# cerbos/cerbos

Measured on NVIDIA H100. Metric: checkresources_decisions_per_sec, higher is better.
Workload: dtype u64

## Files before the change

### cerbos_b200/csrc/cb_core.h

```cpp
#pragma once
#include <stdint.h>
#if !defined(__CUDACC_RTC__)
#include <math.h>
#endif

#include "cerbos_b200_format.h"

#if defined(__CUDACC__)
#define CB_HD __host__ __device__ __forceinline__
#define CB_HD_NOINLINE __host__ __device__ __noinline__
#else
#define CB_HD inline
#define CB_HD_NOINLINE
#endif

namespace cb {

struct alignas(16) U4 { uint32_t x, y, z, w; };

struct TableLayout {
    uint32_t off[32];
    uint32_t nV, nRP, nS, nP, nR, nAP, nT, n_slots, n_rows;
    uint32_t has_role_policies, has_parent_roles, has_principal_policies;
    uint32_t image_bytes;
    uint32_t uc_conds_off, uc_rows_off, uc_chain_off, n_uconds;
    uint32_t theap_words;
    uint32_t uses_runtime;
};

struct TableView {
    const uint8_t *base;
    const TableLayout *L;
    template <typename T>
    CB_HD const T *sec(int id) const { return reinterpret_cast<const T *>(base + L->off[id]); }
    CB_HD const uint32_t *scope_parent() const { return sec<uint32_t>(CB_SEC_SCOPE_PARENT); }
    CB_HD const uint32_t *scope_flags() const { return sec<uint32_t>(CB_SEC_SCOPE_FLAGS); }
    CB_HD const uint32_t *res_block_map() const { return sec<uint32_t>(CB_SEC_RES_BLOCK_MAP); }
    CB_HD const uint8_t *res_exists() const { return sec<uint8_t>(CB_SEC_RES_EXISTS); }
    CB_HD const uint32_t *prin_block_map() const { return sec<uint32_t>(CB_SEC_PRIN_BLOCK_MAP); }
    CB_HD const uint8_t *prin_exists() const { return sec<uint8_t>(CB_SEC_PRIN_EXISTS); }
// ... 9 lines not shown
    CB_HD const uint8_t *str_bytes() const { return sec<uint8_t>(CB_SEC_STR_BYTES); }
    CB_HD const uint32_t *par_off() const { return sec<uint32_t>(CB_SEC_ROLE_PARENTS_OFF); }
    CB_HD const uint32_t *par_list() const { return sec<uint32_t>(CB_SEC_ROLE_PARENTS); }
    CB_HD const uint32_t *rp_off() const { return sec<uint32_t>(CB_SEC_ROLEPOL_OFF); }
    CB_HD const cb_rolepol_entry *rp_entries() const { return sec<cb_rolepol_entry>(CB_SEC_ROLEPOL_ENTRIES); }
    CB_HD const cb_rolepol_rule *rp_rules() const { return sec<cb_rolepol_rule>(CB_SEC_ROLEPOL_RULES); }
    CB_HD const uint32_t *rp_apats() const { return sec<uint32_t>(CB_SEC_ROLEPOL_APATS); }
    CB_HD const uint32_t *block_slots_off() const { return sec<uint32_t>(CB_SEC_BLOCK_SLOTS_OFF); }
    CB_HD const uint32_t *block_slots() const { return sec<uint32_t>(CB_SEC_BLOCK_SLOTS); }
    CB_HD const uint32_t *dr_off() const { return sec<uint32_t>(CB_SEC_DR_OFF); }
    CB_HD const uint32_t *dr_entries() const { return sec<uint32_t>(CB_SEC_DR_ENTRIES); }
    CB_HD const uint32_t *dr_parents() const { return sec<uint32_t>(CB_SEC_DR_PARENTS); }
    CB_HD const uint32_t *dr_name_str() const { return sec<uint32_t>(CB_SEC_DR_NAME_STR); }
    CB_HD const cb_cond *uconds() const { return reinterpret_cast<const cb_cond *>(base + L->uc_conds_off); }
    CB_HD const U4 *urows() const { return reinterpret_cast<const U4 *>(base + L->uc_rows_off); }
    CB_HD const U4 *uc_chain() const { return reinterpret_cast<const U4 *>(base + L->uc_chain_off); }
};

enum { CB_MAX_GATHER = 8 };
struct BatchView {
    const cb_hdr0 *hdr0;
    const cb_hdr1 *hdr1;
    const uint32_t *roles;
    const uint64_t *slots;
    const uint64_t *heap;
    const uint32_t *bstr_off;
    const uint8_t *bstr_bytes;
    const uint32_t *class_off, *class_pats, *aset_k;
    const uint64_t *aset_spread;
    const uint64_t *row_am;
// ... 4223 lines not shown
        for (uint32_t j = 1; j < RC; j++) x |= allow_pairs >> j;
        x &= amask;
        if (RC == 1) acc = x;
        else if (RC == 2) { x = (x | x >> 1) & 0x33333333u; x = (x | x >> 2) & 0x0F0F0F0Fu; x = (x | x >> 4) & 0x00FF00FFu; acc = (x | x >> 8) & 0xFFFFu; }
        else for (uint32_t kk = 0; kk < K; kk++) acc |= ((x >> (kk * RC)) & 1) << kk;
    }
    store_result(b, cols, n, bitmap, effects, K, acc);
    return false;
}

CB_HD U4 uc_row_record(const U4 ur, uint32_t am, uint32_t RCP, uint32_t nR) {
    const uint32_t role = ur.y & 0xFFu, deny = ((ur.y >> 8) & 0xFFu) == CB_EFFECT_DENY;
    U4 r; r.x = am; r.y = ur.z; r.z = ur.w; r.w = (role == 0xFFu ? nR : role) * RCP | deny << 31;
    return r;
}
struct UcRowsGlobal {
    const U4 *urows; const uint64_t *row_am; uint32_t RCP, nR;
    CB_HD U4 get(uint32_t aset_base, uint32_t ri) const { const U4 ur = ld16(urows + ri); return uc_row_record(ur, (uint32_t)ldg(row_am + aset_base + ur.x), RCP, nR); }
};
struct UcRowsPacked {
    const U4 *pk;
    CB_HD U4 get(uint32_t aset_base, uint32_t ri) const { return ld16(pk + aset_base + ri); }
};

struct CachedCols {
    const BatchView *b;
    uint64_t n;
    CB_HD U4 hdr0() const { return ldcol128(b->hdr0 + n); }
    CB_HD uint64_t hdr1() const { return ldcol64(reinterpret_cast<const uint64_t *>(b->hdr1 + n)); }
    CB_HD uint32_t role(uint32_t i) const { return ldcol32(b->roles + (uint64_t)i * b->stride + n); }
    CB_HD uint64_t slot(uint32_t v) const {
#if defined(__CUDA_ARCH__)
        uint64_t x;
        asm("ld.global.nc.u64 %0, [%1];" : "=l"(x) : "l"(b->slots + (uint64_t)v * b->stride + n));
        return x;
#else
        return b->slots[(uint64_t)v * b->stride + n];
#endif
    }
    CB_HD void prefetch_slot(uint32_t) const {}
    CB_HD bool staged() const { return true; }
    CB_HD uint32_t aset_k(uint32_t aset) const { return ldg(b->aset_k + aset); }
    CB_HD const uint64_t *row_am() const { return b->row_am; }
    CB_HD bool stage_result(uint32_t) const { return false; }
};

struct CondWord { uint64_t lo, hi; };
enum { CB_UC_FORM_MASK32 = 0, CB_UC_FORM_MASK64 = 1, CB_UC_FORM_INDEX = 2 };
struct GenericConds {
    static constexpr int kForm = CB_UC_FORM_MASK64;
    static constexpr uint32_t kScopeRows = 0;
    template <typename Cols>
    CB_HD Cols load(const TableView, const BatchView &, const Cols &cols) const { return cols; }
    template <typename Cols>
    CB_HD CondWord operator()(const TableView t, const BatchView &b, const Cols &cols, uint32_t pid, uint64_t n, bool &slow) const {
        if (t.L->n_uconds > 63) { slow = true; CondWord w; w.lo = 1; w.hi = 0; return w; }
        uint64_t val = 1;
        for (uint32_t u = 1, nu = t.L->n_uconds; u <= nu; u++) {
            const U4 cd = ld16(t.uconds() + u);
            uint32_t r;
            if (cd.w) r = flat_dnf_inline(t, b, cols, pid, cd.z, cd.w);
            else r = 4u;
            slow |= (r & 4u) != 0;
            val |= (uint64_t)(r & 1u) << u;
        }
        CondWord w; w.lo = val; w.hi = 0;
        return w;
    }
};

CB_HD uint32_t cond_bit(const CondWord v, uint32_t u) { return (uint32_t)(((u & 64u) ? v.hi : v.lo) >> (u & 63u)) & 1u; }
template <typename RP, int kForm>
CB_HD uint32_t uc_row_pairs(const U4 r, const RP rp, const CondWord v, const uint32_t role_all) {
    const uint32_t vlo = (uint32_t)v.lo, vhi = (uint32_t)(v.lo >> 32);
    const uint32_t miss = kForm == CB_UC_FORM_MASK32   ? r.y & ~vlo
                          : kForm == CB_UC_FORM_MASK64 ? (r.y & ~vlo) | (r.z & ~vhi)
                                                       : (cond_bit(v, r.y & 0xFFu) & cond_bit(v, (r.y >> 8) & 0xFFu)) ^ 1u;
    const uint32_t rc = miss ? 0u : (uint32_t)(rp >> (r.w & (sizeof(RP) * 8 - 1))) & role_all;
    return r.x * rc;
}
constexpr uint32_t kUcUnrollRows = 16;
template <uint32_t kRows, typename RP, int kForm, typename Rows>
CB_HD uint32_t uc_walk(const TableView t, const Rows rows, const RP rp, const CondWord val, const uint32_t r0, const uint32_t bm_base,
                       const uint32_t aset_base, const uint32_t role_all, uint32_t alive) {
    uint32_t allow_pairs = 0;
    const U4 *chain = t.uc_chain() + bm_base;
    for (uint32_t s = r0; s != CB_NONE32 && alive;) {
        const U4 d = ld16(chain + s);
        uint32_t D = 0, A = 0;
        auto row = [&](uint32_t ri) {
            const U4 r = rows.get(aset_base, ri);
            const uint32_t p = uc_row_pairs<RP, kForm>(r, rp, val, role_all), deny = (uint32_t)((int32_t)r.w >> 31);
            D |= p & deny;
            A |= p & ~deny;
        };
        if constexpr (kRows != 0 && kRows <= kUcUnrollRows) {
            if (d.x < d.z) {
                const uint32_t last = d.z - d.x - 1;
#if defined(__CUDA_ARCH__)
#pragma unroll
#endif
                for (uint32_t j = 0; j < kRows; j++) row(d.x + (j < last ? j : last));
            }
        } else {
#if defined(__CUDA_ARCH__)
#pragma unroll 4
#endif
            for (uint32_t ri = d.x; ri < d.z; ri++) row(ri);
        }
        D &= alive;
        alive &= ~D;
        A &= alive;
        allow_pairs |= A;
        alive &= ~A;
        s = d.w;
    }
    return allow_pairs;
}

template <typename Cols, typename Rows, typename Conds = GenericConds>
CB_HD bool eval_request_uc(const TableView t, const BatchView &b, const Cols &cols, const Rows rows, uint64_t n, uint8_t *bitmap, uint8_t *effects,
                           const Conds conds = Conds()) {
    const U4 h0 = cols.hdr0();
// ... 11 lines not shown
        rp |= rr < t.L->nR ? 1ull << (rr * RCP + i) : 0ull;
    }
    if (pv != rv) return true;
    uint32_t acc = 0;
    const bool live = n_roles != 0 && K != 0 && rv != CB_NONE16 && kc != CB_KIND_NONE;
#ifdef CB_UC_STUB_WALK
    const uint32_t r0 = live ? rscope & 0xFFFFu : CB_NONE32;
#else
    const uint32_t r0 = live ? chain_start(t, rscope, CB_SCOPE_FLAG_RESOURCE, (b.flags & CB_BATCH_FLAG_LENIENT) != 0) : CB_NONE32;
#endif
    if (r0 != CB_NONE32) {
        bool slow = false;
        const CondWord val = conds(t, b, regs, pid, n, slow);
        if (slow) return true;
        const uint32_t role_all = (1u << n_roles) - 1;
        const uint32_t aset_base = aset * b.n_rows;
        const uint32_t amask = K * RC >= 32 ? b.stride_pattern : b.stride_pattern & ((1u << (K * RC)) - 1);
        const uint32_t alive0 = amask * role_all;
        const uint32_t bm_base = (rv * t.L->nRP + kc) * t.L->nS;
        uint32_t allow_pairs;
#ifdef CB_UC_STUB_WALK
        allow_pairs = alive0 & ((uint32_t)val.lo ^ (uint32_t)(val.lo >> 32) ^ (uint32_t)rp ^ r0 ^ bm_base ^ aset_base);
        (void)rows;
#else
        if ((t.L->nR + 1) * RCP <= 32)
            allow_pairs = uc_walk<Conds::kScopeRows, uint32_t, Conds::kForm>(t, rows, (uint32_t)rp | role_all << (t.L->nR * RCP), val, r0, bm_base, aset_base, role_all, alive0);
        else allow_pairs = uc_walk<Conds::kScopeRows, uint64_t, Conds::kForm>(t, rows, rp | (uint64_t)role_all << (t.L->nR * RCP), val, r0, bm_base, aset_base, role_all, alive0);
#endif
        uint32_t x = allow_pairs;
        x |= RC > 1 ? allow_pairs >> 1 : 0u;
        x |= RC > 2 ? allow_pairs >> 2 : 0u;
        x |= RC > 3 ? allow_pairs >> 3 : 0u;
        for (uint32_t j = 4; j < RC; j++) x |= allow_pairs >> j;
        x &= amask;
        if (RC == 1) acc = x;
        else if (RC == 2) { x = (x | x >> 1) & 0x33333333u; x = (x | x >> 2) & 0x0F0F0F0Fu; x = (x | x >> 4) & 0x00FF00FFu; acc = (x | x >> 8) & 0xFFFFu; }
        else if (RC == 3) { x = (x | x >> 2) & 0xC30C30C3u; x = (x | x >> 4) & 0x0F00F00Fu; x = (x | x >> 8) & 0xFF0000FFu; acc = (x | x >> 16) & 0x7FFu; }
        else if (RC == 4) { x = (x | x >> 3) & 0x03030303u; x = (x | x >> 6) & 0x000F000Fu; acc = (x | x >> 12) & 0xFFu; }
        else for (uint32_t kk = 0; kk < K; kk++) acc |= ((x >> (kk * RC)) & 1) << kk;
    }
    store_result(b, cols, n, bitmap, effects, K, acc);
    return false;
// ... 13 lines not shown
```

### cerbos_b200/csrc/cb_host.h

```cpp
#pragma once
#include <cstdarg>
#include <cstdint>
#include <cstdio>
#include <cstring>
#include <string>

#include "cb_core.h"
#include "cb_uc.h"
#include "cerbos_b200.h"

namespace cbhost {

constexpr int kMaxSec = 32;

inline std::string msg(const char *fmt, ...) {
    char buf[512];
    va_list ap;
    va_start(ap, fmt);
    vsnprintf(buf, sizeof(buf), fmt, ap);
    va_end(ap);
    return buf;
}

inline std::string parse_blob(const void *blob, size_t len, cb::TableLayout *lay, uint32_t *meta, uint64_t *sec_len) {
// ... 90 lines not shown
    cb::finish_batch_view(*v);
    v->n_bstr = cb_[CGPU_COL_BSTR_OFF] >= 4 ? (uint32_t)(cb_[CGPU_COL_BSTR_OFF] / 4 - 1) : 0;
    v->heap_words = cb_[CGPU_COL_HEAP] / 8;
    return "";
}


inline bool lean_table(const cb::TableLayout &lay, const uint32_t *meta) {
    return !lay.has_principal_policies && !lay.has_role_policies && !lay.has_parent_roles && meta[CB_META_DIRECT_KINDS];
}
inline bool lean_eligible(const cb::TableLayout &lay, const uint32_t *meta, const cb::BatchView &bv) {
    return bv.n_pass == 1 && (uint64_t)bv.max_actions * bv.role_cols <= 32 && bv.kbytes <= 4 && lean_table(lay, meta) &&
           (uint64_t)lay.nR * bv.rcp <= 64;
}
inline bool uc_eligible(const cb::TableLayout &lay, const cbuc::Image &uc, const cb::BatchView &bv) {
    return uc.ok && (uint64_t)(lay.nR + 1) * bv.rcp <= 64 && bv.count < (1ull << 32) && (uint64_t)bv.n_asets * lay.n_rows < (1ull << 31);
}

}
```

### cerbos_b200/csrc/cb_kernels.h

```cpp
#pragma once
#include "cb_core.h"

namespace cbk {

constexpr int kThreads = 256;

struct TableDesc {
    const uint8_t *base;
    cb::TableLayout lay;
};

__device__ __forceinline__ uint32_t smem_u32(const void *p) { return (uint32_t)__cvta_generic_to_shared(p); }

__device__ __forceinline__ void mbar_wait(uint64_t *bar, uint32_t parity) {
    uint32_t ok = 0;
    while (!ok) {
        asm volatile("{\n\t.reg .pred p;\n\tmbarrier.try_wait.parity.shared::cta.b64 p, [%1], %2;\n\tselp.u32 %0, 1, 0, p;\n\t}"
                     : "=r"(ok)
                     : "r"(smem_u32(bar)), "r"(parity)
                     : "memory");
    }
}
__device__ __forceinline__ void mbar_init(uint64_t *bar, uint32_t count) { asm volatile("mbarrier.init.shared::cta.b64 [%0], %1;" ::"r"(smem_u32(bar)), "r"(count)); }
__device__ __forceinline__ void mbar_expect_tx(uint64_t *bar, uint32_t bytes) {
// ... 230 lines not shown
        else if (q < 6 + bv.role_cols) { p = (unsigned long long)(bv.roles + (uint64_t)(q - 6) * bv.stride); sh = 2; }
        else { const uint32_t v = q - 6 - bv.role_cols; p = (unsigned long long)(bv.slots + (uint64_t)(v >> 1) * bv.stride) + (v & 1u) * 128u; sh = 3; }
        pf_base[q] = p;
        pf_shift[q] = sh;
    }
    if (!kStaged) __syncthreads();
    if (kStaged) {
        if (threadIdx.x == 0) {
            mbar_init(mbar, 1);
            asm volatile("fence.mbarrier_init.release.cluster;" ::: "memory");
        }
        __syncthreads();
        if (threadIdx.x == 0) tma_load_image(smem_image, td, mbar);
        mbar_wait(mbar, 0);
        cb::U4 *pks = reinterpret_cast<cb::U4 *>(smem_image + ((td.lay.image_bytes + 127u) & ~127u));
        const uint32_t n_pk = bv.n_asets * bv.n_rows;
        const cb::U4 *ur = tv.urows();
        for (uint32_t j = threadIdx.x; j < n_pk; j += kThreads) {
            const cb::U4 u = ur[j % bv.n_rows];
            pks[j] = cb::uc_row_record(u, (uint32_t)bv.row_am[(j / bv.n_rows) * bv.n_rows + u.x], bv.rcp, td.lay.nR);
        }
        __syncthreads();
        pk = pks;
    }
    const uint32_t lane = threadIdx.x & 31u;
    const uint64_t n_chunks = (bv.count + 31) / 32;
    const uint64_t n_warps = (uint64_t)gridDim.x * (kThreads / 32);
    for (uint64_t chunk = (uint64_t)blockIdx.x * (kThreads / 32) + (threadIdx.x >> 5); chunk < n_chunks; chunk += n_warps) {
        const uint64_t i = chunk * 32 + lane;
        {
            const uint64_t c2 = chunk + n_warps;
            if (c2 * 32 + 32 <= bv.count) {
                const uint64_t n2 = bv.first + c2 * 32;
                for (uint32_t q = lane; q < n_pf; q += 32) asm volatile("prefetch.global.L2 [%0];" ::"l"(pf_base[q] + (n2 << pf_shift[q])));
            }
        }
        if (i < bv.count) {
            const uint64_t n = bv.first + i;
            Cols gc;
            gc.b = &bv; gc.n = n;
            bool d;
            if (kStaged || pk) { cb::UcRowsPacked rows; rows.pk = pk; d = cb::eval_request_uc(tv, bv, gc, rows, n, bitmap, effects, Conds()); }
            else { cb::UcRowsGlobal rows; rows.urows = tv.urows(); rows.row_am = bv.row_am; rows.RCP = bv.rcp; rows.nR = td.lay.nR; d = cb::eval_request_uc(tv, bv, gc, rows, n, bitmap, effects, Conds()); }
            if (d) {
                cb::store_result(bv, gc, n, bitmap, effects, bv.max_actions, 0u);
                const uint32_t k = atomicAdd(bv.defer_count, 1u);
                bv.defer_list[k] = (uint32_t)i;
            }
        }
    }
}

}
```

### cerbos_b200/csrc/cb_specialize.h

```cpp
#pragma once
#include <stdint.h>

#include <cstdio>
#include <cstring>
#include <map>
#include <string>
#include <vector>

#include "cerbos_b200_format.h"

namespace cbspec {

struct Limits {
    uint32_t max_shapes = 8;
    uint32_t max_items = 96;
};

inline std::string hex(uint32_t v) {
    char buf[16];
    snprintf(buf, sizeof buf, "0x%xu", v);
    return buf;
}
inline std::string hex64(uint64_t v) {
    char buf[32];
// ... 374 lines not shown
    uint32_t max_terms = 512;
};
struct UcSource {
    std::string src;
    uint32_t n_strpred = 0;
    uint32_t n_atoms = 0;
};
inline UcSource generate_uc(const uint8_t *uc_image, const uint32_t *off, uint32_t uc_conds_off, uint32_t n_uconds, uint32_t n_slots, uint32_t n_consts = 0,
                            const UcLimits lim = UcLimits()) {
    UcSource out;
    if (n_uconds == 0 || n_uconds > 127) return out;
    const uint32_t *const_words = reinterpret_cast<const uint32_t *>(uc_image + off[CB_SEC_CONSTS]);
    Atoms atoms;
    std::vector<std::string> formula(n_uconds + 1);
    const uint32_t *uconds = reinterpret_cast<const uint32_t *>(uc_image + uc_conds_off);
    const uint32_t scope_rows = uconds[0];
    const uint32_t *code = reinterpret_cast<const uint32_t *>(uc_image + off[CB_SEC_CODE]);
    const uint64_t *consts = reinterpret_cast<const uint64_t *>(uc_image + off[CB_SEC_CONSTS_V64]);
    const uint64_t *theap = reinterpret_cast<const uint64_t *>(uc_image + off[CB_SEC_THEAP]);
    const uint32_t kUseMask = ~((uint32_t)(CB_TERM_LIT_F | CB_TERM_GROUP_END) << 8);
    std::map<std::vector<uint32_t>, uint32_t> term_ids;
    std::vector<std::vector<uint32_t>> terms;
    const uint32_t ns = n_slots ? n_slots : 1;
    std::vector<bool> slot_used(ns, false), slot_list(ns, false);
    auto is_slot_kind = [](uint32_t kind) { return kind == CB_OPK_SLOT || kind == CB_OPK_SLOT_ELEM || kind == CB_OPK_SLOT_SIZE; };
    auto use_slot = [&](uint32_t kind, uint32_t v) { if (is_slot_kind(kind) && v < ns) slot_used[v] = true; };
    auto v64_tag = [](uint64_t b) { const uint32_t top = (uint32_t)(b >> 48); return (top & 0xFFF0u) == 0xFFF0u ? (top & 0xFu) : 0u; };
    for (uint32_t u = 1; u <= n_uconds; u++) {
        const uint32_t *cd = uconds + 4 * u;
        if (cd[3] == 0 || ((cd[3] >> 16) & 0xFF) != CB_FLAT_DNF) {
            formula[u] = translate_program(code, cd[0], cd[1], const_words, n_consts, ns, atoms);
// ... 284 lines not shown
        for (uint32_t v = 0; v < ns; v++) {
            const std::string V = std::to_string(v);
            if (ty[v] == 'S') s += "    ListKey k" + V + ";   // string: its probe key (the id when typed)\n";
            if (ty[v] == 'N') s += "    double d" + V + ";\n";
            if (ty[v] == 'B') s += "    bool b" + V + ";\n";
        }
    }
    for (uint32_t v = 0; v < ns; v++)
        if (slot_list[v]) s += "    ListRegs l" + std::to_string(v) + ";\n";
    s += "    CB_HD uint64_t slot(uint32_t v) const {\n        switch (v) {\n";
    for (uint32_t v = 0; v < ns && !typed; v++)
        if (reg(v)) s += "        case " + std::to_string(v) + "u: return s" + std::to_string(v) + ";\n";
    s += "        default: return v < " + std::to_string(ns) + "u ? g.slot(v) : (uint64_t)(CB_V64_BOX_BASE | CB_V64_ERROR) << 48;\n        }\n    }\n};\n";
    s += "struct SpecConds {\n    static constexpr uint32_t n_strpred = " + std::to_string(n_pred_bits) + "u;\n";
    s += std::string("    static constexpr int kForm = ") + (n_uconds <= 31 ? "CB_UC_FORM_MASK32" : n_uconds <= 63 ? "CB_UC_FORM_MASK64" : "CB_UC_FORM_INDEX") + ";   // how the rows name their conditions\n";
    s += "    static constexpr uint32_t kScopeRows = " + std::to_string(scope_rows) + "u;   // rows of the longest scope (cb::uc_walk)\n";
    s += std::string("    static constexpr bool kPrograms = ") + (have_atoms ? "true" : "false") + ";   // leaf programs: needs the value helpers of cb_core.h\n";
    s += "    template <typename Cols>\n    CB_HD SpecRegs load(const TableView t, const BatchView &b, const Cols &c) const {\n        SpecRegs r;\n        r.g.b = c.b; r.g.n = c.n;\n";
    for (uint32_t v = 0; v < ns; v++)
        if (reg(v)) s += "        r.s" + std::to_string(v) + " = c.slot(" + std::to_string(v) + "u);\n";
    if (typed) {
        std::string guard;
        for (uint32_t v = 0; v < ns; v++) {
            const std::string V = std::to_string(v);
            if (!reg(v)) continue;
            if (ty[v] == 'L') s += "        r.l" + V + " = list_load(t, b, r.s" + V + ");\n";
            if (ty[v] == 'S') s += "        r.k" + V + " = list_probe_key(r.s" + V + ");\n";
            if (ty[v] == 'N') s += "        r.d" + V + " = u2d(r.s" + V + ");\n";
            if (ty[v] == 'B') s += "        r.b" + V + " = (r.s" + V + " & 1u) != 0;\n";
            guard += std::string(guard.empty() ? "" : " & ") + (ty[v] == 'L' ? "typed_list(r.l" + V + ", " + std::to_string(list_need[v]) + "u)"
                                                                 : std::string(ty[v] == 'S' ? "typed_str" : ty[v] == 'N' ? "typed_num" : "typed_bool") + "(r.s" + V + ")");
// ... 117 lines not shown
```

### cerbos_b200/csrc/cb_uc.h

```cpp
#pragma once
#include <stdint.h>

#include <cstring>
#include <map>
#include <string>
#include <tuple>
#include <vector>

#include "cb_core.h"

namespace cbuc {

constexpr uint32_t kMaxUconds = 127;
constexpr uint32_t kMaxMaskUconds = 63;

struct Image {
    bool ok = false;
    std::string why;
    std::vector<uint8_t> bytes;
    cb::TableLayout lay{};
    uint32_t n_uconds = 0, n_flat = 0;
    bool needs_spec() const { return n_flat != n_uconds || n_uconds > kMaxMaskUconds; }
    uint32_t scope_rows = 0;
    uint32_t n_gids = 0, n_gids_flat = 0;
    std::vector<uint32_t> ucond_of_gid;
};

inline Image build(const uint8_t *image, const uint32_t *off, const uint64_t *len, const uint32_t *meta, const cb::TableLayout &lay) {
    Image out;
    const uint32_t n_blocks = meta[CB_META_N_BLOCKS], n_rows = meta[CB_META_N_ROWS], n_conds = meta[CB_META_N_CONDS];
    if (n_blocks == 0) { out.why = "no policy blocks"; return out; }
    if (lay.nR > 64) { out.why = "more than 64 roles"; return out; }
    const uint32_t *blocks = reinterpret_cast<const uint32_t *>(image + off[CB_SEC_BLOCKS]);
    const uint32_t *rows = reinterpret_cast<const uint32_t *>(image + off[CB_SEC_ROWS]);
    const uint32_t *conds = reinterpret_cast<const uint32_t *>(image + off[CB_SEC_CONDS]);
    if (len[CB_SEC_BLOCKS] < (uint64_t)n_blocks * 16 || len[CB_SEC_ROWS] < (uint64_t)n_rows * 16 || len[CB_SEC_CONDS] < (uint64_t)n_conds * 16) {
        out.why = "section sizes do not match META";
        return out;
// ... 50 lines not shown
    const uint64_t n_map = (uint64_t)meta[CB_META_N_VERSIONS] * meta[CB_META_N_RESPATS] * nS;
    if (nS == 0 || len[CB_SEC_SCOPE_PARENT] < (uint64_t)nS * 4 || len[CB_SEC_SCOPE_FLAGS] < (uint64_t)nS * 4 || len[CB_SEC_RES_BLOCK_MAP] < n_map * 4) {
        out.why = "scope tables do not match the block map";
        return out;
    }
    const uint32_t *parent = reinterpret_cast<const uint32_t *>(image + off[CB_SEC_SCOPE_PARENT]);
    const uint32_t *sflags = reinterpret_cast<const uint32_t *>(image + off[CB_SEC_SCOPE_FLAGS]);
    const uint32_t *bmap = reinterpret_cast<const uint32_t *>(image + off[CB_SEC_RES_BLOCK_MAP]);
    std::vector<uint32_t> next(nS);
    for (uint32_t s = 0; s < nS; s++) {
        uint32_t x = s, steps = 0;
        do { x = parent[x]; } while (x != CB_NONE32 && x < nS && ++steps <= nS && !(sflags[x] & CB_SCOPE_FLAG_RESOURCE));
        if (x != CB_NONE32 && (x >= nS || steps > nS)) { out.why = "scope parent chain out of range"; return out; }
        next[s] = x;
    }
    std::vector<uint32_t> chain(4 * (size_t)n_map, 0);
    for (uint64_t e = 0; e < n_map; e++) {
        const uint32_t s = (uint32_t)(e % nS), bid = bmap[e];
        uint32_t *d = chain.data() + 4 * e;
        if (bid != CB_NONE32) {
            if (bid >= n_blocks) { out.why = "block map entry out of range"; return out; }
            const uint32_t *bl = ublocks.data() + 4 * (size_t)bid;
            const bool allow_counts = ((sflags[s] >> CB_SCOPE_PERM_SHIFT) & 3) == 1;
            d[0] = bl[0];
            d[1] = bl[0] + bl[2];
            d[2] = allow_counts ? bl[0] + bl[1] : d[1];
            out.scope_rows = d[2] - d[0] > out.scope_rows ? d[2] - d[0] : out.scope_rows;
        }
        d[3] = next[s];
    }
    ucond_rec[0] = out.scope_rows;
    out.lay = lay;
    for (auto &o : out.lay.off) o = 0;
    auto append = [&](const void *p, uint64_t n) {
        const uint32_t at = (uint32_t)out.bytes.size();
        out.bytes.resize((out.bytes.size() + n + 15) & ~(size_t)15, 0);
        if (n) memcpy(out.bytes.data() + at, p, n);
        return at;
    };
    append("CBUC", 4);
    for (int id : {CB_SEC_SCOPE_PARENT, CB_SEC_SCOPE_FLAGS, CB_SEC_CODE, CB_SEC_CONSTS, CB_SEC_CONSTS_V64, CB_SEC_THEAP,
                   CB_SEC_STR_OFF, CB_SEC_STR_BYTES})
        out.lay.off[id] = append(image + off[id], len[id]);
    out.lay.uc_conds_off = append(ucond_rec.data(), ucond_rec.size() * 4);
    out.lay.uc_rows_off = append(urows.data(), urows.size() * 4);
    out.lay.uc_chain_off = append(chain.data(), chain.size() * 4);
    out.lay.n_uconds = out.n_uconds;
    out.lay.theap_words = (uint32_t)(len[CB_SEC_THEAP] / 8);
    out.lay.image_bytes = (uint32_t)out.bytes.size();
    out.ok = true;
    return out;
}

}
```

### cerbos_b200/csrc/cerbos_b200.cu

```cuda
#include <cuda_runtime.h>
#include <dlfcn.h>
#include <sys/stat.h>
#include <unistd.h>

#include <atomic>
#include <cstdarg>
#include <cstdio>
#include <cstdlib>
#include <cstring>
#include <map>
#include <mutex>
#include <new>
#include <string>
#include <thread>
#include <vector>

#include "cb_core.h"
#include "cb_kernels.h"
#include "cb_specialize.h"
#include "cb_uc.h"
#include "cb_encode.h"
#include "cb_narrow.h"
#include "cb_host.h"
#include "cb_embed.inc"
// ... 137 lines not shown
template <bool kStaged>
__global__ void __launch_bounds__(kThreads, CB_MIN_BLOCKS) check_uc(const __grid_constant__ TableDesc td, const __grid_constant__ cb::BatchView bv, uint8_t *bitmap,
                                                                  uint8_t *effects, uint32_t *status, const uint32_t) {
    extern __shared__ __align__(128) uint8_t smem_image[];
    __shared__ __align__(8) uint64_t mbar;
    (void)status;
    cbk::check_uc_body<cb::GenericConds, cb::CachedCols, kStaged>(td, bv, bitmap, effects, smem_image, &mbar);
}

struct SignalParams { uint32_t *flags[cb::CB_MAX_GATHER]; const uint32_t *wait_flags; uint32_t n_ranks, my_rank, step, wait_step; };
__global__ void __launch_bounds__(kThreads) uc_merge_rows(const __grid_constant__ TableDesc td, const __grid_constant__ cb::BatchView bv, cb::U4 *out, const uint32_t n_pk) {
    const uint32_t j = blockIdx.x * kThreads + threadIdx.x;
    if (j >= n_pk) return;
    cb::TableView tv;
    tv.base = td.base; tv.L = &td.lay;
    const cb::U4 u = tv.urows()[j % bv.n_rows];
    out[j] = cb::uc_row_record(u, (uint32_t)bv.row_am[(j / bv.n_rows) * bv.n_rows + u.x], bv.rcp, td.lay.nR);
}

__global__ void gather_signal(const __grid_constant__ SignalParams p) {
    asm volatile("griddepcontrol.wait;" ::: "memory");
    __threadfence_system();
    if (threadIdx.x < p.n_ranks) asm volatile("red.release.sys.global.max.u32 [%0], %1;" ::"l"(p.flags[threadIdx.x] + p.my_rank), "r"(p.step) : "memory");
    if (p.wait_step) cbk::gather_wait_flags(p.wait_flags, p.n_ranks, p.wait_step);
}
__global__ void gather_wait(const uint32_t *flags, uint32_t n_ranks, uint32_t step) {
    if (threadIdx.x < n_ranks) {
        uint32_t v;
        do {
            asm volatile("ld.acquire.sys.global.u32 %0, [%1];" : "=r"(v) : "l"(flags + threadIdx.x) : "memory");
        } while ((int32_t)(v - step) < 0);
    }
// ... 529 lines not shown
    *list = b.list.ptr;
    *cell = ln.cells + 4 * q;
    *strpred = n_strpred ? b.strpred.ptr : nullptr;
    *pk = n_pk ? b.pk.ptr : nullptr;
    return CGPU_OK;
}

LaunchPlan plan_launch(const cgpu_ctx &ctx, const cgpu_table &t, const cb::BatchView &bv) {
    const cb::TableLayout &lay = t.desc.lay;
    LaunchPlan p;
    p.stage = !ctx.force_no_stage && lay.image_bytes <= kMaxStageBytes;
    const bool spec_ready = t.spec_state.load(std::memory_order_acquire) == 1;
    const bool uc_spec_ready = spec_ready && t.spec_uc_global != nullptr;
    const bool mostly_programs = t.uc.ok && !uc_spec_ready && 2 * (uint64_t)t.uc.n_gids_flat < t.uc.n_gids;
    p.lean = !ctx.force_general && !mostly_programs && cbhost::lean_eligible(lay, t.meta, bv);
    const uint64_t n_pk = (uint64_t)bv.n_asets * lay.n_rows;
    p.uc = p.lean && cbhost::uc_eligible(lay, t.uc, bv) && (uc_spec_ready || !t.uc.needs_spec()) && t.d_uc_image &&
           (ctx.uc_mode == 1 || (ctx.uc_mode != 0 && ctx.cluster_mode != 1 && t.meta[CB_META_BLOCK_SHAPES] > 1));
    p.cluster = !p.uc && bv.count < (1ull << 32) &&
                (ctx.cluster_mode == 1 || (ctx.cluster_mode != 0 && bv.count >= kClusterMinRequests && t.meta[CB_META_BLOCK_SHAPES] > 1));
    const uint32_t tile_bytes = cb::tile_cols_bytes(bv.role_cols, lay.n_slots);
    const uint64_t small_tabs = n_pk * 8 + (((uint64_t)bv.n_asets + 1) & ~1ull) * 4 + 16 + 2 * kThreads;
    const uint32_t tiles_smem = ((lay.image_bytes + 127u) & ~127u) + 2 * tile_bytes + (uint32_t)(small_tabs < 65536 ? small_tabs : 65536);
    auto al16 = [](const void *ptr) { return (reinterpret_cast<uintptr_t>(ptr) & 15) == 0; };
    p.col_tiles = !p.uc && p.lean && p.stage && !p.cluster && !ctx.force_no_tiles && tiles_smem <= kMaxTilesSmem && bv.stride % 4 == 0 &&
                  bv.first % 4 == 0 && al16(bv.hdr0) && al16(bv.hdr1) && al16(bv.roles) && al16(bv.slots);
    p.uc_staged = p.uc && !ctx.force_no_stage && uc_stageable(t.uc, n_pk) && (!uc_spec_ready || t.spec_uc != nullptr);
    p.spec = p.uc ? uc_spec_ready : p.lean && p.stage && bv.count < (1ull << 32) && spec_ready && t.spec_tiles != nullptr;
    p.kernel = p.uc        ? (p.spec ? (p.uc_staged ? Kernel::SpecUc : Kernel::SpecUcGlobal) : p.uc_staged ? Kernel::Uc : Kernel::UcGlobal)
             : p.spec      ? (p.col_tiles ? Kernel::SpecTiles : Kernel::SpecDirect)
             : p.col_tiles ? Kernel::LeanTiles
             : p.lean      ? (p.stage ? Kernel::Lean : Kernel::LeanGlobal)
                           : (p.stage ? Kernel::General : Kernel::GeneralGlobal);
    p.smem = p.uc ? (p.uc_staged ? (uint32_t)uc_smem_bytes(t.uc, n_pk) : 0) : p.col_tiles ? tiles_smem : p.stage ? lay.image_bytes : 0;
    p.last_arg = p.col_tiles ? lay.n_slots : p.stage ? 1u : 0u;
    p.serialise = p.spec && !p.uc && !ctx.profiling;
    p.strpred = p.uc && p.spec && t.spec_n_strpred;
// ... 58 lines not shown
    cb::BatchView bvv = bv;
    bvv.perm = nullptr;
    bvv.prefetch_slots = lay.n_slots <= 8 ? lay.n_slots : 0;
    uint32_t *perm = nullptr;
    if (plan.cluster) {
        int rc = launch_cluster(ctx, t, bv, &perm, stream);
        if (rc != CGPU_OK) return rc;
        bvv.perm = perm;
    }
    uint32_t last_arg = plan.last_arg;
    uint32_t *defer = nullptr;
    if (plan.lean) {
        uint32_t *cell = nullptr, *strpred = nullptr;
        cb::U4 *pk = nullptr;
        const uint32_t n_str = lay.nT + bv.n_bstr;
        const uint64_t n_pk = (uint64_t)bv.n_asets * lay.n_rows;
        int rc = acquire_defer(ctx, stream, bv.count, &defer, &cell, plan.strpred ? (size_t)n_str + 1 : 0, &strpred, plan.merge_rows ? (size_t)n_pk : 0, &pk);
        if (rc != CGPU_OK) return rc;
        if (plan.merge_rows) {
            uc_merge_rows<<<(unsigned)((n_pk + kThreads - 1) / kThreads), kThreads, 0, stream>>>(t->uc_desc, bvv, pk, (uint32_t)n_pk);
            CUDA_TRY(cudaGetLastError());
            ctx->launches.fetch_add(1, std::memory_order_relaxed);
            bvv.uc_rows_pk = pk;
        }
        bvv.defer_count = cell;
        bvv.tile_counter = plan.col_tiles ? cell + 2 : nullptr;
        bvv.defer_list = defer;
        if (plan.strpred && n_str) {
            TableDesc ptd = t->uc_desc;
            uint32_t n_arg = n_str;
            void *pargs[] = {&ptd, &bvv, &strpred, &n_arg};
// ... 913 lines not shown
```

Measured before the change: 87.60 billion.

## Lay out unconditional rows as fixed deny/allow slot segments per block

Builds a padded per-block slot table that splits each block's rows into a fixed-size deny segment and a fixed-size allow segment. The walk can then use compile-time trip counts with full unrolling and no per-row deny-bit branching. Allow-versus-deny handling moves into per-scope masks stored in the chain. The packed per-aset row records are pre-merged by slot, so staged kernels index them directly. The cost is padding: empty slots are still evaluated, and the packed tables get larger.

Result: faster. 90.88 billion, median of 6 (+3.7%).

```diff
diff --git a/cerbos_b200/csrc/cb_core.h b/cerbos_b200/csrc/cb_core.h
--- a/cerbos_b200/csrc/cb_core.h
+++ b/cerbos_b200/csrc/cb_core.h
@@ -24,6 +24,9 @@
     uint32_t has_role_policies, has_parent_roles, has_principal_policies;
     uint32_t image_bytes;
     uint32_t uc_conds_off, uc_rows_off, uc_chain_off, n_uconds;
+    uint32_t uc_n_rows;
+    uint32_t uc_slots_off;
+    uint32_t uc_deny_rows, uc_allow_rows;
     uint32_t theap_words;
     uint32_t uses_runtime;
 };
@@ -63,6 +66,7 @@
     CB_HD const uint32_t *dr_name_str() const { return sec<uint32_t>(CB_SEC_DR_NAME_STR); }
     CB_HD const cb_cond *uconds() const { return reinterpret_cast<const cb_cond *>(base + L->uc_conds_off); }
     CB_HD const U4 *urows() const { return reinterpret_cast<const U4 *>(base + L->uc_rows_off); }
+    CB_HD const uint32_t *uc_slots() const { return reinterpret_cast<const uint32_t *>(base + L->uc_slots_off); }
     CB_HD const U4 *uc_chain() const { return reinterpret_cast<const U4 *>(base + L->uc_chain_off); }
 };
 
@@ -4316,13 +4320,41 @@
     U4 r; r.x = am; r.y = ur.z; r.z = ur.w; r.w = (role == 0xFFu ? nR : role) * RCP | deny << 31;
     return r;
 }
+CB_HD U4 uc_slot_record(const U4 r, bool used) {
+    U4 z; z.x = used ? r.x : 0u; z.y = r.y; z.z = r.z; z.w = r.w & 0x7FFFFFFFu;
+    return z;
+}
 struct UcRowsGlobal {
     const U4 *urows; const uint64_t *row_am; uint32_t RCP, nR;
-    CB_HD U4 get(uint32_t aset_base, uint32_t ri) const { const U4 ur = ld16(urows + ri); return uc_row_record(ur, (uint32_t)ldg(row_am + aset_base + ur.x), RCP, nR); }
+    const uint32_t *slots = nullptr;
+    CB_HD UcRowsGlobal aset(const TableView t, const BatchView &b, uint32_t a) const {
+        UcRowsGlobal r = *this;
+        r.row_am += (uint64_t)a * b.n_rows;
+        r.slots = t.uc_slots();
+        return r;
+    }
+    CB_HD UcRowsGlobal at(uint32_t first) const { UcRowsGlobal r = *this; r.slots += first; return r; }
+    CB_HD U4 get(uint32_t ri) const { const U4 ur = ld16(urows + ri); return uc_row_record(ur, (uint32_t)ldg(row_am + ur.x), RCP, nR); }
+    CB_HD U4 slot(uint32_t j) const { const uint32_t ri = ldg(slots + j); return uc_slot_record(get(ri != CB_NONE32 ? ri : 0u), ri != CB_NONE32); }
+    CB_HD U4 merged(const TableView t, uint32_t j) const { return t.L->uc_slots_off ? slot(j) : get(j); }
 };
 struct UcRowsPacked {
     const U4 *pk;
-    CB_HD U4 get(uint32_t aset_base, uint32_t ri) const { return ld16(pk + aset_base + ri); }
+    bool by_slot = false;
+    const uint32_t *slots = nullptr;
+    CB_HD UcRowsPacked aset(const TableView t, const BatchView &b, uint32_t a) const {
+        UcRowsPacked r = *this;
+        r.pk = pk + a * (by_slot ? t.L->uc_n_rows : b.n_rows);
+        r.slots = t.uc_slots();
+        return r;
+    }
+    CB_HD UcRowsPacked at(uint32_t first) const { UcRowsPacked r = *this; if (by_slot) r.pk += first; else r.slots += first; return r; }
+    CB_HD U4 get(uint32_t ri) const { return ld16(pk + ri); }
+    CB_HD U4 slot(uint32_t j) const {
+        if (by_slot) return ld16(pk + j);
+        const uint32_t ri = ldg(slots + j);
+        return uc_slot_record(ld16(pk + (ri != CB_NONE32 ? ri : 0u)), ri != CB_NONE32);
+    }
 };
 
 struct CachedCols {
@@ -4349,9 +4381,11 @@
 
 struct CondWord { uint64_t lo, hi; };
 enum { CB_UC_FORM_MASK32 = 0, CB_UC_FORM_MASK64 = 1, CB_UC_FORM_INDEX = 2 };
+constexpr uint32_t kUcUnrollRows = 16;
+constexpr uint32_t kUcRowsOfLayout = ~0u;
 struct GenericConds {
     static constexpr int kForm = CB_UC_FORM_MASK64;
-    static constexpr uint32_t kScopeRows = 0;
+    static constexpr uint32_t kDenyRows = kUcRowsOfLayout, kAllowRows = kUcRowsOfLayout;
     template <typename Cols>
     CB_HD Cols load(const TableView, const BatchView &, const Cols &cols) const { return cols; }
     template <typename Cols>
@@ -4373,42 +4407,48 @@
 
 CB_HD uint32_t cond_bit(const CondWord v, uint32_t u) { return (uint32_t)(((u & 64u) ? v.hi : v.lo) >> (u & 63u)) & 1u; }
 template <typename RP, int kForm>
-CB_HD uint32_t uc_row_pairs(const U4 r, const RP rp, const CondWord v, const uint32_t role_all) {
+CB_HD uint32_t uc_row_pairs(const U4 r, const RP rp, const CondWord v, const uint32_t role_all, const uint32_t shift) {
     const uint32_t vlo = (uint32_t)v.lo, vhi = (uint32_t)(v.lo >> 32);
     const uint32_t miss = kForm == CB_UC_FORM_MASK32   ? r.y & ~vlo
                           : kForm == CB_UC_FORM_MASK64 ? (r.y & ~vlo) | (r.z & ~vhi)
                                                        : (cond_bit(v, r.y & 0xFFu) & cond_bit(v, (r.y >> 8) & 0xFFu)) ^ 1u;
-    const uint32_t rc = miss ? 0u : (uint32_t)(rp >> (r.w & (sizeof(RP) * 8 - 1))) & role_all;
+    const uint32_t rc = miss ? 0u : (uint32_t)(rp >> shift) & role_all;
     return r.x * rc;
 }
-constexpr uint32_t kUcUnrollRows = 16;
-template <uint32_t kRows, typename RP, int kForm, typename Rows>
+template <uint32_t kDenyRows, uint32_t kAllowRows, typename RP, int kForm, typename Rows>
 CB_HD uint32_t uc_walk(const TableView t, const Rows rows, const RP rp, const CondWord val, const uint32_t r0, const uint32_t bm_base,
-                       const uint32_t aset_base, const uint32_t role_all, uint32_t alive) {
+                       const uint32_t role_all, uint32_t alive) {
+    constexpr bool kOfLayout = kDenyRows == kUcRowsOfLayout;
+    const uint32_t n_deny = kOfLayout ? t.L->uc_deny_rows : kDenyRows, n_allow = kOfLayout ? t.L->uc_allow_rows : kAllowRows;
+    const bool segments = n_deny + n_allow != 0;
     uint32_t allow_pairs = 0;
     const U4 *chain = t.uc_chain() + bm_base;
     for (uint32_t s = r0; s != CB_NONE32 && alive;) {
         const U4 d = ld16(chain + s);
         uint32_t D = 0, A = 0;
-        auto row = [&](uint32_t ri) {
-            const U4 r = rows.get(aset_base, ri);
-            const uint32_t p = uc_row_pairs<RP, kForm>(r, rp, val, role_all), deny = (uint32_t)((int32_t)r.w >> 31);
-            D |= p & deny;
-            A |= p & ~deny;
-        };
-        if constexpr (kRows != 0 && kRows <= kUcUnrollRows) {
-            if (d.x < d.z) {
-                const uint32_t last = d.z - d.x - 1;
+        if (segments) {
+            const Rows seg = rows.at(d.x);
+            auto slot = [&](uint32_t j) { const U4 r = seg.slot(j); return uc_row_pairs<RP, kForm>(r, rp, val, role_all, r.w); };
 #if defined(__CUDA_ARCH__)
 #pragma unroll
 #endif
-                for (uint32_t j = 0; j < kRows; j++) row(d.x + (j < last ? j : last));
-            }
+            for (uint32_t j = 0; j < n_deny; j++) D |= slot(j);
+#if defined(__CUDA_ARCH__)
+#pragma unroll
+#endif
+            for (uint32_t j = 0; j < n_allow; j++) A |= slot(n_deny + j);
+            D |= A & d.z;
+            A &= d.y;
         } else {
 #if defined(__CUDA_ARCH__)
 #pragma unroll 4
 #endif
-            for (uint32_t ri = d.x; ri < d.z; ri++) row(ri);
+            for (uint32_t ri = d.x; ri < d.z; ri++) {
+                const U4 r = rows.get(ri);
+                const uint32_t p = uc_row_pairs<RP, kForm>(r, rp, val, role_all, r.w & (sizeof(RP) * 8 - 1)), deny = (uint32_t)((int32_t)r.w >> 31);
+                D |= p & deny;
+                A |= p & ~deny;
+            }
         }
         D &= alive;
         alive &= ~D;
@@ -4450,18 +4490,18 @@
         const CondWord val = conds(t, b, regs, pid, n, slow);
         if (slow) return true;
         const uint32_t role_all = (1u << n_roles) - 1;
-        const uint32_t aset_base = aset * b.n_rows;
         const uint32_t amask = K * RC >= 32 ? b.stride_pattern : b.stride_pattern & ((1u << (K * RC)) - 1);
         const uint32_t alive0 = amask * role_all;
         const uint32_t bm_base = (rv * t.L->nRP + kc) * t.L->nS;
         uint32_t allow_pairs;
 #ifdef CB_UC_STUB_WALK
-        allow_pairs = alive0 & ((uint32_t)val.lo ^ (uint32_t)(val.lo >> 32) ^ (uint32_t)rp ^ r0 ^ bm_base ^ aset_base);
+        allow_pairs = alive0 & ((uint32_t)val.lo ^ (uint32_t)(val.lo >> 32) ^ (uint32_t)rp ^ r0 ^ bm_base ^ aset);
         (void)rows;
 #else
+        const Rows arows = rows.aset(t, b, aset);
         if ((t.L->nR + 1) * RCP <= 32)
-            allow_pairs = uc_walk<Conds::kScopeRows, uint32_t, Conds::kForm>(t, rows, (uint32_t)rp | role_all << (t.L->nR * RCP), val, r0, bm_base, aset_base, role_all, alive0);
-        else allow_pairs = uc_walk<Conds::kScopeRows, uint64_t, Conds::kForm>(t, rows, rp | (uint64_t)role_all << (t.L->nR * RCP), val, r0, bm_base, aset_base, role_all, alive0);
+            allow_pairs = uc_walk<Conds::kDenyRows, Conds::kAllowRows, uint32_t, Conds::kForm>(t, arows, (uint32_t)rp | role_all << (t.L->nR * RCP), val, r0, bm_base, role_all, alive0);
+        else allow_pairs = uc_walk<Conds::kDenyRows, Conds::kAllowRows, uint64_t, Conds::kForm>(t, arows, rp | (uint64_t)role_all << (t.L->nR * RCP), val, r0, bm_base, role_all, alive0);
 #endif
         uint32_t x = allow_pairs;
         x |= RC > 1 ? allow_pairs >> 1 : 0u;
diff --git a/cerbos_b200/csrc/cb_host.h b/cerbos_b200/csrc/cb_host.h
--- a/cerbos_b200/csrc/cb_host.h
+++ b/cerbos_b200/csrc/cb_host.h
@@ -128,7 +128,8 @@
            (uint64_t)lay.nR * bv.rcp <= 64;
 }
 inline bool uc_eligible(const cb::TableLayout &lay, const cbuc::Image &uc, const cb::BatchView &bv) {
-    return uc.ok && (uint64_t)(lay.nR + 1) * bv.rcp <= 64 && bv.count < (1ull << 32) && (uint64_t)bv.n_asets * lay.n_rows < (1ull << 31);
+    return uc.ok && (uint64_t)(lay.nR + 1) * bv.rcp <= 64 && bv.count < (1ull << 32) && (uint64_t)bv.n_asets * lay.n_rows < (1ull << 31) &&
+           (uint64_t)bv.n_asets * uc.lay.uc_n_rows < (1ull << 31);
 }
 
 }
diff --git a/cerbos_b200/csrc/cb_kernels.h b/cerbos_b200/csrc/cb_kernels.h
--- a/cerbos_b200/csrc/cb_kernels.h
+++ b/cerbos_b200/csrc/cb_kernels.h
@@ -268,12 +268,9 @@
         if (threadIdx.x == 0) tma_load_image(smem_image, td, mbar);
         mbar_wait(mbar, 0);
         cb::U4 *pks = reinterpret_cast<cb::U4 *>(smem_image + ((td.lay.image_bytes + 127u) & ~127u));
-        const uint32_t n_pk = bv.n_asets * bv.n_rows;
-        const cb::U4 *ur = tv.urows();
-        for (uint32_t j = threadIdx.x; j < n_pk; j += kThreads) {
-            const cb::U4 u = ur[j % bv.n_rows];
-            pks[j] = cb::uc_row_record(u, (uint32_t)bv.row_am[(j / bv.n_rows) * bv.n_rows + u.x], bv.rcp, td.lay.nR);
-        }
+        const uint32_t n_u = td.lay.uc_n_rows, n_pk = bv.n_asets * n_u;
+        cb::UcRowsGlobal g; g.urows = tv.urows(); g.row_am = bv.row_am; g.RCP = bv.rcp; g.nR = td.lay.nR;
+        for (uint32_t j = threadIdx.x; j < n_pk; j += kThreads) pks[j] = g.aset(tv, bv, j / n_u).merged(tv, j % n_u);
         __syncthreads();
         pk = pks;
     }
@@ -294,7 +291,7 @@
             Cols gc;
             gc.b = &bv; gc.n = n;
             bool d;
-            if (kStaged || pk) { cb::UcRowsPacked rows; rows.pk = pk; d = cb::eval_request_uc(tv, bv, gc, rows, n, bitmap, effects, Conds()); }
+            if (kStaged || pk) { cb::UcRowsPacked rows; rows.pk = pk; rows.by_slot = true; d = cb::eval_request_uc(tv, bv, gc, rows, n, bitmap, effects, Conds()); }
             else { cb::UcRowsGlobal rows; rows.urows = tv.urows(); rows.row_am = bv.row_am; rows.RCP = bv.rcp; rows.nR = td.lay.nR; d = cb::eval_request_uc(tv, bv, gc, rows, n, bitmap, effects, Conds()); }
             if (d) {
                 cb::store_result(bv, gc, n, bitmap, effects, bv.max_actions, 0u);
diff --git a/cerbos_b200/csrc/cb_specialize.h b/cerbos_b200/csrc/cb_specialize.h
--- a/cerbos_b200/csrc/cb_specialize.h
+++ b/cerbos_b200/csrc/cb_specialize.h
@@ -412,7 +412,7 @@
     Atoms atoms;
     std::vector<std::string> formula(n_uconds + 1);
     const uint32_t *uconds = reinterpret_cast<const uint32_t *>(uc_image + uc_conds_off);
-    const uint32_t scope_rows = uconds[0];
+    const uint32_t scope_rows = uconds[0], deny_rows = uconds[1], allow_rows = uconds[2];
     const uint32_t *code = reinterpret_cast<const uint32_t *>(uc_image + off[CB_SEC_CODE]);
     const uint64_t *consts = reinterpret_cast<const uint64_t *>(uc_image + off[CB_SEC_CONSTS_V64]);
     const uint64_t *theap = reinterpret_cast<const uint64_t *>(uc_image + off[CB_SEC_THEAP]);
@@ -727,7 +727,9 @@
     s += "        default: return v < " + std::to_string(ns) + "u ? g.slot(v) : (uint64_t)(CB_V64_BOX_BASE | CB_V64_ERROR) << 48;\n        }\n    }\n};\n";
     s += "struct SpecConds {\n    static constexpr uint32_t n_strpred = " + std::to_string(n_pred_bits) + "u;\n";
     s += std::string("    static constexpr int kForm = ") + (n_uconds <= 31 ? "CB_UC_FORM_MASK32" : n_uconds <= 63 ? "CB_UC_FORM_MASK64" : "CB_UC_FORM_INDEX") + ";   // how the rows name their conditions\n";
-    s += "    static constexpr uint32_t kScopeRows = " + std::to_string(scope_rows) + "u;   // rows of the longest scope (cb::uc_walk)\n";
+    s += "    static constexpr uint32_t kScopeRows = " + std::to_string(scope_rows) + "u;   // rows the walk visits per scope (cb::uc_walk)\n";
+    s += "    static constexpr uint32_t kDenyRows = " + std::to_string(deny_rows) + "u, kAllowRows = " + std::to_string(allow_rows) +
+         "u;   // segment slots (0 / 0: row ranges)\n";
     s += std::string("    static constexpr bool kPrograms = ") + (have_atoms ? "true" : "false") + ";   // leaf programs: needs the value helpers of cb_core.h\n";
     s += "    template <typename Cols>\n    CB_HD SpecRegs load(const TableView t, const BatchView &b, const Cols &c) const {\n        SpecRegs r;\n        r.g.b = c.b; r.g.n = c.n;\n";
     for (uint32_t v = 0; v < ns; v++)
diff --git a/cerbos_b200/csrc/cb_uc.h b/cerbos_b200/csrc/cb_uc.h
--- a/cerbos_b200/csrc/cb_uc.h
+++ b/cerbos_b200/csrc/cb_uc.h
@@ -22,6 +22,7 @@
     uint32_t n_uconds = 0, n_flat = 0;
     bool needs_spec() const { return n_flat != n_uconds || n_uconds > kMaxMaskUconds; }
     uint32_t scope_rows = 0;
+    uint32_t deny_rows = 0, allow_rows = 0;
     uint32_t n_gids = 0, n_gids_flat = 0;
     std::vector<uint32_t> ucond_of_gid;
 };
@@ -102,22 +103,60 @@
         if (x != CB_NONE32 && (x >= nS || steps > nS)) { out.why = "scope parent chain out of range"; return out; }
         next[s] = x;
     }
+    std::vector<uint8_t> used(n_blocks, 0);
+    for (uint64_t e = 0; e < n_map; e++) {
+        const uint32_t bid = bmap[e];
+        if (bid == CB_NONE32) continue;
+        if (bid >= n_blocks) { out.why = "block map entry out of range"; return out; }
+        used[bid] |= 1 | (((sflags[e % nS] >> CB_SCOPE_PERM_SHIFT) & 3) == 1) << 1;
+    }
+    uint32_t max_deny = 0, max_allow = 0, max_deny_only = 0;
+    for (uint32_t b = 0; b < n_blocks; b++) {
+        const uint32_t *bl = ublocks.data() + 4 * (size_t)b;
+        if (used[b] & 2) {
+            max_deny = bl[2] > max_deny ? bl[2] : max_deny;
+            max_allow = bl[1] - bl[2] > max_allow ? bl[1] - bl[2] : max_allow;
+        } else if (used[b]) max_deny_only = bl[2] > max_deny_only ? bl[2] : max_deny_only;
+    }
+    if (max_deny_only > max_deny + max_allow) max_allow = max_deny_only - max_deny;
+    const uint32_t seg = max_deny + max_allow;
+    const bool segments = seg >= 1 && seg <= cb::kUcUnrollRows && ((uint64_t)n_blocks + 1) * seg < (1ull << 31);
+    std::vector<uint32_t> slots;
+    if (segments) {
+        out.deny_rows = max_deny;
+        out.allow_rows = max_allow;
+        slots.assign(((size_t)n_blocks + 1) * seg, CB_NONE32);
+        for (uint32_t b = 0; b < n_blocks; b++) {
+            const uint32_t *bl = ublocks.data() + 4 * (size_t)b;
+            const uint32_t n_use = (used[b] & 2) ? bl[1] : used[b] ? bl[2] : 0;
+            for (uint32_t r = 0; r < n_use; r++)
+                slots[(size_t)(b + 1) * seg + (r < bl[2] || !(used[b] & 2) ? r : max_deny + r - bl[2])] = bl[0] + r;
+        }
+    }
     std::vector<uint32_t> chain(4 * (size_t)n_map, 0);
     for (uint64_t e = 0; e < n_map; e++) {
         const uint32_t s = (uint32_t)(e % nS), bid = bmap[e];
         uint32_t *d = chain.data() + 4 * e;
         if (bid != CB_NONE32) {
-            if (bid >= n_blocks) { out.why = "block map entry out of range"; return out; }
             const uint32_t *bl = ublocks.data() + 4 * (size_t)bid;
             const bool allow_counts = ((sflags[s] >> CB_SCOPE_PERM_SHIFT) & 3) == 1;
-            d[0] = bl[0];
-            d[1] = bl[0] + bl[2];
-            d[2] = allow_counts ? bl[0] + bl[1] : d[1];
-            out.scope_rows = d[2] - d[0] > out.scope_rows ? d[2] - d[0] : out.scope_rows;
+            if (segments) {
+                d[0] = (bid + 1) * seg;
+                d[1] = allow_counts ? ~0u : 0u;
+                d[2] = (used[bid] & 2) ? 0u : ~0u;
+            } else {
+                d[0] = bl[0];
+                d[1] = bl[0] + bl[2];
+                d[2] = allow_counts ? bl[0] + bl[1] : d[1];
+                out.scope_rows = d[2] - d[0] > out.scope_rows ? d[2] - d[0] : out.scope_rows;
+            }
         }
         d[3] = next[s];
     }
+    if (segments) out.scope_rows = seg;
     ucond_rec[0] = out.scope_rows;
+    ucond_rec[1] = out.deny_rows;
+    ucond_rec[2] = out.allow_rows;
     out.lay = lay;
     for (auto &o : out.lay.off) o = 0;
     auto append = [&](const void *p, uint64_t n) {
@@ -133,7 +172,11 @@
     out.lay.uc_conds_off = append(ucond_rec.data(), ucond_rec.size() * 4);
     out.lay.uc_rows_off = append(urows.data(), urows.size() * 4);
     out.lay.uc_chain_off = append(chain.data(), chain.size() * 4);
+    out.lay.uc_slots_off = segments ? append(slots.data(), slots.size() * 4) : 0;
     out.lay.n_uconds = out.n_uconds;
+    out.lay.uc_n_rows = segments ? (uint32_t)slots.size() : (uint32_t)(urows.size() / 4);
+    out.lay.uc_deny_rows = out.deny_rows;
+    out.lay.uc_allow_rows = out.allow_rows;
     out.lay.theap_words = (uint32_t)(len[CB_SEC_THEAP] / 8);
     out.lay.image_bytes = (uint32_t)out.bytes.size();
     out.ok = true;
diff --git a/cerbos_b200/csrc/cerbos_b200.cu b/cerbos_b200/csrc/cerbos_b200.cu
--- a/cerbos_b200/csrc/cerbos_b200.cu
+++ b/cerbos_b200/csrc/cerbos_b200.cu
@@ -175,8 +175,9 @@
     if (j >= n_pk) return;
     cb::TableView tv;
     tv.base = td.base; tv.L = &td.lay;
-    const cb::U4 u = tv.urows()[j % bv.n_rows];
-    out[j] = cb::uc_row_record(u, (uint32_t)bv.row_am[(j / bv.n_rows) * bv.n_rows + u.x], bv.rcp, td.lay.nR);
+    const uint32_t n_u = td.lay.uc_n_rows;
+    cb::UcRowsGlobal g; g.urows = tv.urows(); g.row_am = bv.row_am; g.RCP = bv.rcp; g.nR = td.lay.nR;
+    out[j] = g.aset(tv, bv, j / n_u).merged(tv, j % n_u);
 }
 
 __global__ void gather_signal(const __grid_constant__ SignalParams p) {
@@ -736,13 +737,13 @@
     const bool uc_spec_ready = spec_ready && t.spec_uc_global != nullptr;
     const bool mostly_programs = t.uc.ok && !uc_spec_ready && 2 * (uint64_t)t.uc.n_gids_flat < t.uc.n_gids;
     p.lean = !ctx.force_general && !mostly_programs && cbhost::lean_eligible(lay, t.meta, bv);
-    const uint64_t n_pk = (uint64_t)bv.n_asets * lay.n_rows;
+    const uint64_t n_pk = (uint64_t)bv.n_asets * t.uc.lay.uc_n_rows;
     p.uc = p.lean && cbhost::uc_eligible(lay, t.uc, bv) && (uc_spec_ready || !t.uc.needs_spec()) && t.d_uc_image &&
            (ctx.uc_mode == 1 || (ctx.uc_mode != 0 && ctx.cluster_mode != 1 && t.meta[CB_META_BLOCK_SHAPES] > 1));
     p.cluster = !p.uc && bv.count < (1ull << 32) &&
                 (ctx.cluster_mode == 1 || (ctx.cluster_mode != 0 && bv.count >= kClusterMinRequests && t.meta[CB_META_BLOCK_SHAPES] > 1));
     const uint32_t tile_bytes = cb::tile_cols_bytes(bv.role_cols, lay.n_slots);
-    const uint64_t small_tabs = n_pk * 8 + (((uint64_t)bv.n_asets + 1) & ~1ull) * 4 + 16 + 2 * kThreads;
+    const uint64_t small_tabs = (uint64_t)bv.n_asets * lay.n_rows * 8 + (((uint64_t)bv.n_asets + 1) & ~1ull) * 4 + 16 + 2 * kThreads;
     const uint32_t tiles_smem = ((lay.image_bytes + 127u) & ~127u) + 2 * tile_bytes + (uint32_t)(small_tabs < 65536 ? small_tabs : 65536);
     auto al16 = [](const void *ptr) { return (reinterpret_cast<uintptr_t>(ptr) & 15) == 0; };
     p.col_tiles = !p.uc && p.lean && p.stage && !p.cluster && !ctx.force_no_tiles && tiles_smem <= kMaxTilesSmem && bv.stride % 4 == 0 &&
@@ -831,7 +832,7 @@
         uint32_t *cell = nullptr, *strpred = nullptr;
         cb::U4 *pk = nullptr;
         const uint32_t n_str = lay.nT + bv.n_bstr;
-        const uint64_t n_pk = (uint64_t)bv.n_asets * lay.n_rows;
+        const uint64_t n_pk = (uint64_t)bv.n_asets * t->uc.lay.uc_n_rows;
         int rc = acquire_defer(ctx, stream, bv.count, &defer, &cell, plan.strpred ? (size_t)n_str + 1 : 0, &strpred, plan.merge_rows ? (size_t)n_pk : 0, &pk);
         if (rc != CGPU_OK) return rc;
         if (plan.merge_rows) {
```
